# MihailMihov/simd-raytracer

Hardware: AMD Instinct MI355X
Metric: Mrays/s (intersect invocations per second), hw09/scene5 dragon 1920x1080 1spp (higher is better)
Workload: dtype f32; 1 GPU; BASELINE configs[1]: scenes/hw09/scene5.crtscene 1920x1080 1spp max_ray_depth=5 (primary + shadow + reflection rays), kd_tree_simd_accel semantics; rays_per_frame=2726485, primary_rays=2073600, parallelism=bucket-tiles x1

## Files before the change

### simd-raytracer_amd/csrc/accel.hpp

```cpp
#pragma once

#include <hip/hip_runtime.h>

#include <cstdlib>
#include <mutex>
#include <string>
#include <vector>

#include "abi_guard.hpp"
#include "kernels.hpp"
#include "stream.hpp"
#include "build.hpp"
#include "dev_mem.hpp"
#include "frame_plan.hpp"
#include "order_judge.hpp"
#include "update_plan.hpp"

struct rtk_knobs {
    uint32_t slice_min_tris = rtk::kSliceMinTrisDefault;
    bool shadow_exit = true;
    bool skip_unlit_shadow = true;
    bool bundle_cull = true;
    bool auto_trials = true;
    bool cost_feedback = true;
// ... 24 lines not shown
    int stream_batch = 0;
    int stream_mem_gb = 96;
    int stream_side_below = 2;
    bool first_frame_prior = true;
    bool fast_occluders = true;
    bool camera_keeps_order = false;
    size_t views_launch_units = 131072;
    bool traversal_fast = false;
    size_t adaptive_chunk_pixels = size_t(1) << 20;

    static rtk_knobs from_env() {
        rtk_knobs k;
        auto geti = [](const char *name, long &out) { const char *e = std::getenv(name); if (!e || !*e) return false; out = std::atol(e); return true; };
        long v;
        if (geti("RTK_SLICE_MIN_TRIS", v) && v > 0) k.slice_min_tris = uint32_t(v);
        if (geti("RTK_SHADOW_EARLY_EXIT", v)) k.shadow_exit = v != 0;
        if (geti("RTK_SKIP_UNLIT_SHADOW", v)) k.skip_unlit_shadow = v != 0;
        if (geti("RTK_BUNDLE_CULL", v)) k.bundle_cull = v != 0;
        if (geti("RTK_AUTO_TRIALS", v)) k.auto_trials = v != 0;
        if (geti("RTK_COST_FEEDBACK", v)) k.cost_feedback = v != 0;
        if (geti("RTK_COST_RESORT_EVERY", v) && v > 0) { k.resort_every = unsigned(v); k.resort_max = 0; }
        if (geti("RTK_COST_RESORT_MAX", v) && v >= 0 && v <= (1l << 30)) k.resort_max = unsigned(v);
        if (geti("RTK_COST_JUDGE", v)) k.judge = v != 0;
        if (geti("RTK_COST_JUDGE_FORCE", v) && v >= rtk::kJudgeByScore && v <= rtk::kJudgeAlwaysKeep) k.judge_force = int(v);
        if (geti("RTK_LIGHT_BELOW_CYCLES", v) && v >= 0) k.light_cycles = uint32_t(v);
        if (geti("RTK_ORDER_FLOOR_CYCLES", v) && v >= 0) k.order_floor_cycles = uint32_t(v);
        if (geti("RTK_REPACK", v)) k.repack = v != 0;
        if (geti("RTK_RASTER_TILES", v)) k.raster_tiles = v != 0;
        if (geti("RTK_REPACK_FULL_BOUNDS", v)) k.repack_full_bounds = v != 0;
        if (geti("RTK_REPACK_SKIP_BITS2", v) && v >= 0 && v <= 22) k.repack_skip_bits2 = int(v);
        if (geti("RTK_REPACK_DIRS3", v)) k.repack_dirs3 = v != 0;
        if (geti("RTK_REPACK_SKIP_BITS", v) && v >= 0 && v <= 14) k.repack_skip_bits = int(v);
        if (geti("RTK_STREAM_SCALAR_SURV", v)) k.stream_scalar_surv = v != 0;
        if (geti("RTK_BATCH_SCALAR_SURV", v)) k.batch_scalar_surv = v != 0;
        if (geti("RTK_REPACK_TRACE", v) && (v == RTK_TRACE_AUTO || v == RTK_TRACE_WAVE || v == RTK_TRACE_LANE)) k.repack_trace = int(v);
        if (geti("RTK_GROUP8_BELOW_BLOCKS", v) && v >= 0) k.group8_below = size_t(v);
        if (geti("RTK_STREAM_NODE_FACTOR", v) && v >= 1) k.stream_node_factor = int(v);
        if (geti("RTK_STREAM_DEEP_LEVEL", v)) k.stream_deep_level = int(v);
        if (geti("RTK_STREAM_DEEP_MODE", v)) k.stream_deep_mode = int(v);
        if (geti("RTK_AUTO_MIN_LANES", v) && v > 0 && v <= 64) k.auto_min_lanes = uint32_t(v);
        if (geti("RTK_STREAM_SORT_FROM", v)) k.stream_sort_from = int(v);
        if (geti("RTK_STREAM_DEBUG", v)) k.stream_debug = v != 0;
        if (geti("RTK_STREAM_SIDE", v)) k.stream_side = v != 0;
        if (geti("RTK_TRAVERSAL_FAST", v)) k.traversal_fast = v != 0;
        if (geti("RTK_FIRST_FRAME_PRIOR", v)) k.first_frame_prior = v != 0;
        if (geti("RTK_STREAM_SLICES", v) && (v == 0 || v == 1 || v == 2 || v == 4)) k.stream_slices = int(v);
        if (geti("RTK_STREAM_BATCH", v) && v >= 0 && v <= 4096) k.stream_batch = int(v);
// ... 330 lines not shown
```

### simd-raytracer_amd/csrc/api_frame.hip

```cpp
#include <cmath>
#include <cstdio>
#include <cstring>
#include <mutex>

#include "accel.hpp"
#include "stream_plan.hpp"

namespace rtk {

int frame_geom(const rtk_accel *a, const rtk_render_params *p, FrameGeom &g) {
    if (!a || !p) return fail(RTK_ERR_INVALID, "null accel or params");
    const int64_t w = p->width > 0 ? p->width : a->scene.width;
    const int64_t h = p->height > 0 ? p->height : a->scene.height;
    if (w <= 0 || h <= 0 || w > 65536 || h > 65536) return fail(RTK_ERR_INVALID, "image size must be in [1, 65536]");
    if (p->spp < 1) return fail(RTK_ERR_INVALID, "spp must be >= 1");
    if (p->max_ray_depth < 0 || p->max_ray_depth > kMaxRayDepth)
        return fail(RTK_ERR_INVALID, "max_ray_depth must be in [0, 16]");
    if (p->diffuse_rays < 0 || p->diffuse_rays > 32767) return fail(RTK_ERR_INVALID, "diffuse_rays must be in [0, 32767]");
    if (!valid_frame_mode(p->trace_mode)) return fail(RTK_ERR_INVALID, "unknown trace_mode");
    if (p->sample_begin < 0 || p->sample_count < 0 || p->sample_begin >= p->spp ||
        int64_t(p->sample_begin) + p->sample_count > p->spp)
        return fail(RTK_ERR_INVALID, "sample_begin / sample_count must select samples inside [0, spp)");
    if (p->sample_count == 0 && p->sample_begin != 0) return fail(RTK_ERR_INVALID, "sample_count == 0 means all samples: sample_begin must be 0");
    g.sample_begin = p->sample_begin;
// ... 257 lines not shown
    }
    RTK_TRY(join_lanes(a, lanes, s));
    S.ws = a->ws;
    RTK_HIP_AS(launch_stream_overflow_reset(S, s), "launch overflow reset");
    dev::RenderArgs F = A;
    F.only_if = a->ws.ctrl + dev::kCtrlOverflow;
    RTK_HIP_AS(launch_render(F, RTK_TRACE_GROUP4, p->collect_stats != 0, general, s), "launch fallback k_render");
    RTK_TRY(release_stream_ws(a, s));
    if (a->knobs.stream_debug) {
        uint32_t h[dev::kCtrlWords];
        (void)hipStreamSynchronize(s);
        (void)hipMemcpy(h, a->ws.ctrl, sizeof(h), hipMemcpyDeviceToHost);
        std::fprintf(stderr, "[rtk stream] node_cap %u hit_cap %u overflow %u; nodes per level:", a->ws.node_cap, a->ws.hit_cap, h[dev::kCtrlOverflow]);
        for (int l = 0; l <= p->max_ray_depth + 1; ++l) std::fprintf(stderr, " %u", l == 0 ? unsigned(n_root) : h[dev::kCtrlNodeCount + l]);
        std::fprintf(stderr, "; hits:");
        for (int l = 0; l <= p->max_ray_depth; ++l) std::fprintf(stderr, " %u", h[dev::kCtrlHitCount + l]);
        std::fprintf(stderr, "\n");
    }
    return RTK_OK;
}

int ensure_feedback_ws(rtk_accel *a, rtk_cost_feedback &fb, const FrameGeom &g, size_t units, hipStream_t s) {
    if (fb.judge.get() == nullptr) {
        RTK_MEM(fb.judge.reserve(kJudgeWords));
        RTK_HIP(hipMemsetAsync(fb.judge.get(), 0, kJudgeWords * sizeof(uint32_t), s));
    }
    if (fb.state.units >= units) return RTK_OK;
    const uint32_t bk = g.bucket;
    const uint64_t tx = (uint64_t(a->scene.width > 0 ? a->scene.width : 0) + bk - 1) / bk, ty = (uint64_t(a->scene.height > 0 ? a->scene.height : 0) + bk - 1) / bk;
    const size_t cap = fb.state.capacity(units, &fb == &a->fb, g.blocks_of(tx * ty));
    RTK_MEM(fb.cost.reserve(cap));
    RTK_MEM(fb.order.reserve(2 * (2 * cap + 4) + 8));
    RTK_MEM(fb.bins.reserve(cap));
    fb.state.units = cap;
    return RTK_OK;
}

struct ListSet { uint32_t *order, *hdr, *wg_list; };
ListSet list_set(rtk_cost_feedback &fb, int k, size_t units) {
    uint32_t *const order = fb.order.get() + size_t(k) * (2 * fb.state.units + 4);
    return {order, order + units, order + units + 4};
}

int read_back_count(rtk_cost_feedback &fb, const ListSet &L, hipStream_t s) {
    RTK_MEM(fb.nwgs_host.reserve(1));
    RTK_MEM(fb.nwgs_ev.ensure());
    RTK_HIP(hipMemcpyAsync(fb.nwgs_host.get(), L.hdr, sizeof(uint32_t), hipMemcpyDeviceToHost, s));
    RTK_HIP(hipEventRecord(fb.nwgs_ev.get(), s));
    return RTK_OK;
}

int launch_sort(rtk_accel *a, rtk_cost_feedback &fb, int k, int frame_mode, size_t units, hipStream_t s, int champion) {
    const ListSet L = list_set(fb, k, units);
    RTK_HIP_AS(launch_order_by_cost(fb.cost.get(), fb.bins.get(), L.order, L.wg_list, L.hdr, uint32_t(units),
                                    frame_mode == RTK_TRACE_GROUP4 ? a->knobs.light_cycles >> 4 : 0u, a->knobs.order_floor_cycles >> 4, 4u, s,
                                    a->knobs.judge ? fb.judge.get() : nullptr, champion),
               "launch k_order_by_cost");
    fb.sorts += 1;
    return read_back_count(fb, L, s);
}

int launch_judge(rtk_accel *a, rtk_cost_feedback &fb, int read_set, size_t units, hipStream_t s) {
    const ListSet R = list_set(fb, read_set, units), O = list_set(fb, read_set ^ 1, units);
    RTK_HIP_AS(launch_judge_order(fb.judge.get(), R.order, O.order, uint32_t(2 * units + 4), a->knobs.judge_force, s), "launch k_judge_order");
    fb.judges += 1;
    fb.state.rearm_count();
    return read_back_count(fb, R, s);
}

int order_launch(rtk_accel *a, rtk_cost_feedback &fb, const rtk_render_params *p, const FrameGeom &g, dev::RenderArgs &A, int frame_mode,
                 size_t units, hipStream_t s, OrderState::Step &step) {
    uint64_t sig[5];
    shape_sig(g, p->spp, p->max_ray_depth, p->diffuse_rays, sig);
    sig[3] = (uint64_t(uint32_t(g.bucket)) << 32) | (uint64_t(uint32_t(g.sample_end - g.sample_begin) & 0xFFFFu) << 16) | uint32_t(p->trace_mode);
    sig[4] = A.regions ? ((1ull << 63) | (uint64_t(A.n_regions) << 32) | uint64_t(A.n_units))
                       : (A.views ? uint64_t(A.n_views) : 0ull);
    RTK_TRY(ensure_feedback_ws(a, fb, g, units, s));
    step = fb.state.step(sig, frame_mode, p->collect_stats != 0, A.regions != nullptr,
                         {a->knobs.first_frame_prior, a->knobs.resort_every, a->knobs.resort_max});
    fb.list_units = units;
    const ListSet L = list_set(fb, step.read_set, units);
    if (step.prior)
        RTK_HIP_AS(launch_block_prior(A, fb.bins.get(), L.order, L.wg_list, L.hdr,
                                      reinterpret_cast<uint32_t *>(A.counters + kPriorScratchWord), 4u, s), "launch k_block_prior");
    if (step.sort_front) RTK_TRY(launch_sort(a, fb, step.read_set, frame_mode, units, s, kChampionNone));
    if (step.use_order) { A.order_in = L.order; A.order_hdr = L.hdr; A.wg_list = L.wg_list; }
    if (&fb == &a->fb) a->cnt.after_order(step);
    A.cost_out = fb.cost.get();
    return RTK_OK;
}

int render_megakernel(rtk_accel *a, rtk_cost_feedback &fb, const rtk_render_params *p, const FrameGeom &g, dev::RenderArgs &A, bool general,
                      hipStream_t s) {
    const size_t units = A.regions ? size_t(A.n_units) : (A.views ? g.blocks() * A.n_views : g.blocks());
    A.n_units = uint32_t(units);
    const int frame_mode = OrderState::frame_mode(p->trace_mode, units, a->knobs.group8_below);
    OrderState::Step step = {};
    if (a->knobs.cost_feedback && units > 0 && units <= 0x7FFFFFFFull) {
        const int rc = order_launch(a, fb, p, g, A, frame_mode, units, s, step);
        if (rc != RTK_OK) { fb.forget(); return rc; }
    }
    unsigned n_wgs = 0;
    if (A.wg_list != nullptr) {
        bool ready = false;
        if (fb.state.awaits_count() && !(ready = hipEventQuery(fb.nwgs_ev.get()) == hipSuccess)) (void)hipGetLastError();
        n_wgs = fb.state.workgroups(ready, fb.nwgs_host.get());
    }
    int rc = RTK_OK;
    const bool judged = step.judge && a->knobs.judge && units <= 0x7FFFFFF0ull / 2;
    if (a->knobs.judge && (judged || step.sort_behind)) {
        n_wgs = 0;
        const hipError_t es = launch_stamp(fb.judge.get(), s);
        if (es != hipSuccess) rc = hip_fail(es, "launch k_stamp");
    }
    const hipError_t e = rc == RTK_OK ? launch_render(A, frame_mode, p->collect_stats != 0, general, s, n_wgs) : hipSuccess;
    if (e != hipSuccess) rc = hip_fail(e, "launch k_render");
    if (rc == RTK_OK && judged) rc = launch_judge(a, fb, step.read_set, units, s);
    if (rc == RTK_OK && step.sort_behind)
        rc = launch_sort(a, fb, step.write_set, frame_mode, units, s, judged ? kChampionLeave : kChampionScore);
    if (rc != RTK_OK) fb.forget();
    return rc;
}

}

dev::RenderArgs frame_args(const rtk_accel *a, const rtk_render_params *p, const FrameGeom &g, const rtk_view &cam, float *d_out) {
    dev::RenderArgs A = scene_args(a, p->collect_stats);
    camera_args(cam, p, g, A);
    A.max_depth = p->max_ray_depth; A.diffuse_rays = p->diffuse_rays;
    A.gi_div_f = static_cast<float>(p->diffuse_rays + 1);
    A.sample_begin = g.sample_begin; A.sample_end = g.sample_end;
    A.shadow_bias = p->shadow_bias; A.reflection_bias = p->reflection_bias; A.refraction_bias = p->refraction_bias;
    A.bucket = g.bucket; A.tiles_x = g.tiles_x; A.tiles_y = g.tiles_y; A.n_buckets = g.n_buckets;
    A.blocks_per_bucket_side = g.blocks_side; A.buckets_per_rank = g.buckets_per_rank;
    A.rank = g.rank; A.world = g.world; A.compact = g.world > 1 ? 1 : 0; A.skew_q = g.skew_q;
    A.out = d_out; A.counters = counters_now(a);
    return A;
}

namespace {

int render_frame_body(rtk_accel *a, const rtk_render_params *p, const FrameGeom &g, const rtk_view &cam, float *d_out, hipStream_t s, bool steady) {
// ... 588 lines not shown
```

### simd-raytracer_amd/csrc/frame_plan.hpp

```cpp
#pragma once

#include <cstddef>
#include <cstdint>
#include <cstring>

#include "../../include/rtk.h"

namespace rtk {

struct FrameGeom {
    uint32_t width, height, bucket, tiles_x, tiles_y, n_buckets, blocks_side, buckets_per_rank;
    uint32_t skew_q;
    int rank, world;
    int sample_begin, sample_end;
    uint64_t blocks_of(uint64_t buckets) const { return buckets * blocks_side * blocks_side; }
    size_t blocks() const { return size_t(blocks_of(buckets_per_rank)); }
};

inline void shape_sig(const FrameGeom &g, int spp, int max_ray_depth, int diffuse_rays, uint64_t out[3]) {
    out[0] = (uint64_t(uint32_t(g.width)) << 32) | uint32_t(g.height);
    out[1] = (uint64_t(uint32_t(g.rank)) << 32) | uint32_t(g.world);
    out[2] = (uint64_t(uint32_t(spp)) << 32) | (uint64_t(uint32_t(max_ray_depth)) << 16) | uint32_t(diffuse_rays);
}

// ... 3 lines not shown
    uint64_t sig[3] = {0, 0, 0};
    int state = 0;

    static bool applies(int trace_mode, bool forks, bool stats) { return trace_mode == RTK_TRACE_AUTO && forks && !stats; }
    bool same(const uint64_t s[3]) const { return std::memcmp(s, sig, sizeof(sig)) == 0; }
    bool waiting(const uint64_t s[3]) const { return state == 3 && same(s); }
    void verdict(float t_stream, float t_mega) { state = t_mega < t_stream ? 5 : 4; }
    void abandon() { state = 0; }
    Step next(const uint64_t s[3], bool trials_on) {
        if (!same(s)) { std::memcpy(sig, s, sizeof(sig)); state = 0; }
        if (!trials_on) return {true, kNoRecord};
        switch (state) {
            case 0: state = 1; return {true, kPipelinePair};
            case 1: state = 2; return {false, kNoRecord};
            case 2: state = 3; return {false, kMegakernelPair};
            case 5: return {false, kNoRecord};
            default: return {true, kNoRecord};
        }
    }
};

struct OrderState {
    struct Knobs { bool first_frame_prior; unsigned resort_every; unsigned resort_max = 0; };
    struct Step { bool prior, resort, use_order, sort_front, sort_behind; int read_set, write_set; bool judge = false; };
    size_t units = 0;
    uint64_t sig[5] = {0, 0, 0, 0, 0};
    bool valid = false;
    bool order_valid = false;
    unsigned age = 0;
    bool nwgs_pending = false, nwgs_known = false;
    int set = 0;
    bool presorted = false;
    unsigned sorts = 0;

    void forget() { valid = false; order_valid = false; age = 0; nwgs_pending = false; nwgs_known = false; set = 0; presorted = false; sorts = 0; }

    void restart_schedule(unsigned resort_every) {
        sorts = 0;
        if (!presorted && resort_every > 0 && age >= resort_every) age = resort_every - 1;
    }

    unsigned interval(const Knobs &k) const {
        uint64_t iv = k.resort_every;
        for (unsigned i = 3; i <= sorts && iv < k.resort_max; ++i) iv *= 2;
        return (k.resort_max > k.resort_every && iv > k.resort_max) ? k.resort_max : unsigned(iv);
    }

    static int frame_mode(int trace_mode, size_t n_units, size_t group8_below) {
        if (trace_mode == RTK_TRACE_TWOPASS) return RTK_TRACE_GROUP4;
        return trace_mode != RTK_TRACE_AUTO ? trace_mode : (n_units < group8_below ? RTK_TRACE_GROUP8 : RTK_TRACE_GROUP4);
    }

    size_t capacity(size_t n_units, bool is_frame_table, uint64_t native) {
        if (units >= n_units) return units;
        size_t cap = n_units;
        if (is_frame_table && units == 0 && native > cap && native <= (1ull << 24)) cap = size_t(native);
        units = 0; valid = false; order_valid = false;
        return cap;
    }

    Step step(const uint64_t s[5], int mode, bool stats, bool regions, const Knobs &k) {
        const bool same_shape = valid && std::memcmp(s, sig, sizeof(sig)) == 0;
        if (!same_shape) { order_valid = false; set = 0; presorted = false; sorts = 0; }
        Step r = {!same_shape && k.first_frame_prior && mode == RTK_TRACE_GROUP4 && !stats && !regions, false, false, false, false, 0, 0, false};
        if (same_shape) {
            r.resort = !order_valid || age >= interval(k);
            if (r.resort) {
                r.sort_front = !presorted;
                r.judge = presorted;
                if (presorted) set ^= 1;
                presorted = false;
                order_valid = true; age = 0; nwgs_known = false; nwgs_pending = true;
                sorts += 1;
            }
            age += 1;
            r.sort_behind = age >= interval(k);
            presorted = r.sort_behind;
        }
        r.use_order = r.prior || same_shape;
        r.read_set = set; r.write_set = set ^ 1;
        std::memcpy(sig, s, sizeof(sig));
        valid = true;
        return r;
    }

    void rearm_count() { if (order_valid) { nwgs_pending = true; nwgs_known = false; } }

    bool awaits_count() const { return order_valid && nwgs_pending; }
    unsigned workgroups(bool ready, const uint32_t *host_word) {
        if (!order_valid) return 0;
        if (nwgs_pending && ready) { nwgs_pending = false; nwgs_known = true; }
        return nwgs_known && !nwgs_pending ? *host_word : 0;
    }
};

struct CounterState {
    struct Step { int current; bool fill, carry; };
    int current = 0;
    bool other_zero = false;
    const void *stream = nullptr;
// ... 40 lines not shown
```

### simd-raytracer_amd/csrc/kernels.hip

```cpp
#include <hip/hip_runtime.h>

#include "kernels.hpp"
#include "order_judge.hpp"
#include "trace.hip.hpp"
#include "shade.hip.hpp"

namespace rtk {
namespace dev {

template <int MODE, bool STATS, bool LDS_NODES>
__global__ __launch_bounds__(256) void k_intersect(IntersectArgs A) {
    extern __shared__ __attribute__((aligned(16))) unsigned char smem[];
    DevNode *lds_nodes = reinterpret_cast<DevNode *>(smem);
    if (LDS_NODES) stage_nodes(A.tree.nodes, A.tree.n_nodes, lds_nodes);

    const size_t slot = (size_t)blockIdx.x * blockDim.x + threadIdx.x;
    const bool active = slot < A.n;
    size_t i = (active && A.perm != nullptr) ? (size_t)A.perm[slot] : slot;
    uint32_t raster_w = A.raster_w;
    if (A.verdict != nullptr) {
        if (A.verdict[16] != 0u) return;
        raster_w = A.verdict[15];
        if (raster_w < 64u || (raster_w & 7u) != 0u || (size_t)raster_w * 16u > A.n) raster_w = 0u;
    }
// ... 866 lines not shown
    const unsigned long long a = acc[i], c = cur[i];
    acc[i] = longest ? (a < c ? c : a) : a + c;
}
}

hipError_t launch_counters_fold(const unsigned long long *cur, unsigned long long *acc, hipStream_t s) {
    hipLaunchKernelGGL(dev::k_counters_fold, dim3(1), dim3(256), 0, s, cur, acc);
    return hipGetLastError();
}

namespace dev {
__device__ __forceinline__ uint32_t cost_bin(uint32_t c) {
    c |= 1u;
    const uint32_t e = 31u - (uint32_t)__clz((int)c);
    const uint32_t m = e >= 3u ? (c >> (e - 3u)) & 7u : (c << (3u - e)) & 7u;
    return e * 8u + m;
}
__global__ __launch_bounds__(1024) void k_order_by_cost(const uint32_t *cost, uint8_t *bins, uint32_t *order, uint32_t *wg_list,
                                                        uint32_t *hdr, uint32_t n, uint32_t light_below, uint32_t floor_below,
                                                        uint32_t pack, uint32_t *judge, int champion) {
    if (judge != nullptr && threadIdx.x == 0u) {
        const unsigned long long now = __builtin_amdgcn_s_memrealtime();
        const unsigned long long t0 = *reinterpret_cast<const unsigned long long *>(judge + kJudgeStampLo);
        if (champion != kChampionLeave) judge[kJudgeChampion] = champion == kChampionScore ? judge_score(t0, now) : 0u;
    }
    __shared__ uint32_t hist[256];
    __shared__ uint32_t start[256];
    __shared__ uint32_t wg_hist[2][256], wg_base[2][256];
    __shared__ uint32_t n_single_sh;
    const uint32_t light_bin = light_below > 0u ? cost_bin(light_below) : 0u;
    const uint32_t floor_raw = floor_below > 0u ? cost_bin(floor_below) : 0u;
    const uint32_t floor_bin = floor_raw < light_bin ? floor_raw : light_bin;
    constexpr uint32_t kBatch = 8;
    for (uint32_t i = threadIdx.x; i < 256u; i += blockDim.x) { hist[i] = 0u; wg_hist[0][i] = 0u; wg_hist[1][i] = 0u; }
    __syncthreads();
    for (uint32_t base = 0; base < n; base += blockDim.x * kBatch) {
        uint32_t c[kBatch];
#pragma unroll
        for (uint32_t k = 0; k < kBatch; ++k) {
            const uint32_t i = base + k * blockDim.x + threadIdx.x;
            c[k] = i < n ? cost[i] : 0u;
        }
#pragma unroll
        for (uint32_t k = 0; k < kBatch; ++k) {
            const uint32_t i = base + k * blockDim.x + threadIdx.x;
            uint32_t b = i < n ? cost_bin(c[k]) : 0u;
            if (b < floor_bin) b = 0u;
// ... 66 lines not shown
    __syncthreads();
    for (uint32_t w = threadIdx.x; w < n_wgs; w += blockDim.x) {
        const bool packed = w >= n_single;
        const uint32_t at = packed ? n_single + (w - n_single) * pack : w;
        const uint32_t blk = order[at];
        uint32_t key = (uint32_t)bins[blk];
        if (packed && key != 0u) key = key + 8u < 255u ? key + 8u : 255u;
        const uint32_t pos = atomicAdd(&wg_base[packed ? 1 : 0][key], 1u);
        wg_list[pos] = packed ? (0x80000000u | at) : blk;
    }
}
}

hipError_t launch_order_by_cost(const uint32_t *cost, uint8_t *bins, uint32_t *order, uint32_t *wg_list, uint32_t *hdr, uint32_t n,
                                uint32_t light_below, uint32_t floor_below, uint32_t pack, hipStream_t s, uint32_t *judge, int champion) {
    if (n == 0u) return hipSuccess;
    if (pack == 0u) return hipErrorInvalidValue;
    hipLaunchKernelGGL(dev::k_order_by_cost, dim3(1), dim3(1024), 0, s, cost, bins, order, wg_list, hdr, n, light_below, floor_below, pack,
                       judge, champion);
    return hipGetLastError();
}

namespace dev {
__global__ __launch_bounds__(64) void k_stamp(unsigned long long *stamp) {
    if (threadIdx.x == 0u) *stamp = __builtin_amdgcn_s_memrealtime();
}
}

hipError_t launch_stamp(uint32_t *judge, hipStream_t s) {
    if (judge == nullptr) return hipErrorInvalidValue;
    hipLaunchKernelGGL(dev::k_stamp, dim3(1), dim3(64), 0, s, reinterpret_cast<unsigned long long *>(judge + kJudgeStampLo));
    return hipGetLastError();
}

namespace dev {
__global__ __launch_bounds__(1024) void k_judge_order(uint32_t *judge, uint32_t *read_set, const uint32_t *other_set, uint32_t words, int force) {
    __shared__ uint32_t take_sh;
    if (threadIdx.x == 0u) {
        const unsigned long long now = __builtin_amdgcn_s_memrealtime();
        const unsigned long long t0 = *reinterpret_cast<const unsigned long long *>(judge + kJudgeStampLo);
        const Verdict v = judge_order({judge[kJudgeChampion], judge_score(t0, now)}, force);
        judge[kJudgeChampion] = v.after.champion;
        judge[kJudgeChallenger] = v.after.challenger;
        judge[v.take ? kJudgeTaken : kJudgeRejected] += 1u;
        take_sh = v.take ? 1u : 0u;
    }
    __syncthreads();
    if (take_sh != 0u) return;
    uint32_t done = 0u;
    if (((reinterpret_cast<uintptr_t>(read_set) | reinterpret_cast<uintptr_t>(other_set)) & 15u) == 0u) {
        const uint32_t quads = words >> 2;
        const uint4 *src = reinterpret_cast<const uint4 *>(other_set);
        uint4 *dst = reinterpret_cast<uint4 *>(read_set);
        constexpr uint32_t kBatch = 4;
        for (uint32_t base = 0; base < quads; base += blockDim.x * kBatch) {
            uint4 v[kBatch];
#pragma unroll
            for (uint32_t k = 0; k < kBatch; ++k) {
                const uint32_t i = base + k * blockDim.x + threadIdx.x;
                if (i < quads) v[k] = src[i];
            }
#pragma unroll
            for (uint32_t k = 0; k < kBatch; ++k) {
                const uint32_t i = base + k * blockDim.x + threadIdx.x;
                if (i < quads) dst[i] = v[k];
            }
        }
        done = quads << 2;
    }
    for (uint32_t i = done + threadIdx.x; i < words; i += blockDim.x) read_set[i] = other_set[i];
}
}

hipError_t launch_judge_order(uint32_t *judge, uint32_t *read_set, const uint32_t *other_set, uint32_t words, int force, hipStream_t s) {
    if (judge == nullptr || read_set == nullptr || other_set == nullptr || read_set == other_set) return hipErrorInvalidValue;
    if (words == 0u) return hipSuccess;
    hipLaunchKernelGGL(dev::k_judge_order, dim3(1), dim3(1024), 0, s, judge, read_set, other_set, words, force);
    return hipGetLastError();
}

hipError_t launch_camera_rays(const dev::RenderArgs &A, int sample, rtk_ray *d_rays, hipStream_t s) {
    const size_t n = (size_t)A.width * A.height;
    if (n == 0) return hipSuccess;
    hipLaunchKernelGGL(dev::k_camera_rays, dim3((unsigned)((n + 255) / 256)), dim3(256), 0, s, A, sample, d_rays);
    return hipGetLastError();
}

hipError_t launch_region_rays(const dev::RenderArgs &A, int sample, uint64_t first, uint32_t n, rtk_ray *d_rays, uint32_t *d_ids, hipStream_t s) {
    if (n == 0u) return hipSuccess;
    if (A.regions == nullptr || A.n_regions == 0u) return hipErrorInvalidValue;
    hipLaunchKernelGGL(dev::k_region_rays, dim3((n + 255u) / 256u), dim3(256), 0, s, A, sample, first, n, d_rays, d_ids);
    return hipGetLastError();
}

hipError_t launch_region_accumulate(const dev::RenderArgs &A, uint64_t first, uint32_t n, const float *d_rgb, bool start, bool divide, hipStream_t s) {
    if (n == 0u) return hipSuccess;
    if (A.regions == nullptr || A.n_regions == 0u) return hipErrorInvalidValue;
    hipLaunchKernelGGL(dev::k_region_accumulate, dim3((n + 255u) / 256u), dim3(256), 0, s, A, first, n, d_rgb, start ? 1 : 0, divide ? 1 : 0);
    return hipGetLastError();
}
// ... 29 lines not shown
```

### simd-raytracer_amd/csrc/kernels.hpp

```cpp
#pragma once

#include <hip/hip_runtime.h>

#include "rtk_internal.hpp"
#include "counters.hpp"

namespace rtk {

constexpr int kMaxRayDepth = 16;
constexpr unsigned long long kCriticalMinTicks = 1000;
constexpr uint32_t kSliceMinTrisDefault = 33;
constexpr size_t kMaxNodeLdsBytes = 48 * 1024;

}

#include "trace.hip.hpp"
#include "regions_plan.hpp"

namespace rtk {
namespace dev {

__host__ __device__ inline uint32_t rank_bucket(uint32_t rank, uint32_t local, uint32_t world, uint32_t skew_q) {
    if (skew_q == 0u) return rank + local * world;
    const uint32_t by = local / skew_q, m = local % skew_q;
// ... 64 lines not shown
    const RegionEntry *regions;
    uint32_t n_regions;

    __device__ __forceinline__ size_t out_index(uint32_t local_bucket, uint32_t lx, uint32_t ly, uint32_t px,
                                                uint32_t py) const {
        return compact ? (((size_t)local_bucket * bucket + ly) * bucket + lx) : ((size_t)py * width + px);
    }
};

struct AssembleArgs {
    const float *gathered;
    float *rgb;
    uint32_t width, height, bucket, tiles_x, world, buckets_per_rank, skew_q;
};

}

hipError_t launch_intersect(const dev::IntersectArgs &A, int mode, bool stats, hipStream_t s);
hipError_t launch_render(const dev::RenderArgs &A, int mode, bool stats, bool forks, hipStream_t s, unsigned n_workgroups = 0);
enum : int { kChampionNone = 0, kChampionScore = 1, kChampionLeave = 2 };
hipError_t launch_order_by_cost(const uint32_t *cost, uint8_t *bins , uint32_t *order, uint32_t *wg_list ,
                                uint32_t *hdr , uint32_t n, uint32_t light_below, uint32_t floor_below, uint32_t pack,
                                hipStream_t s, uint32_t *judge = nullptr, int champion = kChampionNone);
hipError_t launch_stamp(uint32_t *judge, hipStream_t s);
hipError_t launch_judge_order(uint32_t *judge, uint32_t *read_set, const uint32_t *other_set, uint32_t words, int force, hipStream_t s);
hipError_t launch_block_prior(const dev::RenderArgs &A, uint8_t *cls, uint32_t *order, uint32_t *wg_list, uint32_t *hdr,
                              uint32_t *scratch, uint32_t pack, hipStream_t s);
hipError_t launch_counters_fold(const unsigned long long *cur, unsigned long long *acc, hipStream_t s);
hipError_t launch_assemble(const dev::AssembleArgs &A, hipStream_t s);
hipError_t launch_camera_rays(const dev::RenderArgs &A, int sample, rtk_ray *d_rays, hipStream_t s);
hipError_t launch_to_rgb8(const float *d_rgb, size_t n, uint8_t *d_out, hipStream_t s);
hipError_t launch_frame_to_texels(const float *d_rgb, size_t n, uint8_t *d_out, hipStream_t s);
hipError_t launch_region_rays(const dev::RenderArgs &A, int sample, uint64_t first, uint32_t n, rtk_ray *d_rays, uint32_t *d_ids, hipStream_t s);
hipError_t launch_region_accumulate(const dev::RenderArgs &A, uint64_t first, uint32_t n, const float *d_rgb, bool start, bool divide, hipStream_t s);
hipError_t launch_add_word(unsigned long long *dst, const unsigned long long *src, hipStream_t s);

}
```

### simd-raytracer_amd/csrc/order_judge.hpp

```cpp
#pragma once

#include <cstdint>

#if defined(__HIPCC__) || defined(__CUDACC__)
#define RTK_JUDGE_FN __host__ __device__ inline
#else
#define RTK_JUDGE_FN inline
#endif

namespace rtk {

enum : int { kJudgeByScore = 0, kJudgeAlwaysTake = 1, kJudgeAlwaysKeep = 2 };

enum : uint32_t {
    kJudgeStampLo = 0, kJudgeStampHi = 1,
    kJudgeChampion = 2,
    kJudgeChallenger = 3,
    kJudgeTaken = 4, kJudgeRejected = 5,
    kJudgeWords = 6
};

RTK_JUDGE_FN uint32_t judge_score(uint64_t frame_start, uint64_t behind_start) {
    if (frame_start == 0 || behind_start <= frame_start) return 0u;
    const uint64_t d = behind_start - frame_start;
    return d > 0xFFFFFFFFull ? 0xFFFFFFFFu : uint32_t(d);
}

struct JudgeScores { uint32_t champion, challenger; };
struct Verdict {
    bool take;
    JudgeScores after;
};

RTK_JUDGE_FN Verdict judge_order(JudgeScores s, int force) {
    bool take = s.champion == 0u || s.challenger == 0u || s.challenger <= s.champion;
    if (force == kJudgeAlwaysTake) take = true;
    if (force == kJudgeAlwaysKeep) take = false;
    return {take, {take ? s.challenger : s.champion, s.challenger}};
}

}
```

### simd-raytracer_amd/csrc/phases.hip.hpp

```cpp
#pragma once

#include <hip/hip_runtime.h>

#include <cstdint>

namespace rtk {
namespace dev {

enum PhaseSlot : int {
    PH_TOTAL = 0,
    PH_TRACE, PH_N_TRACE,
    PH_STEPS,
    PH_N_SMALL, PH_T_SMALL, PH_C_SMALL,
    PH_N_BIG, PH_T_BIG, PH_C_BIG,
    PH_PROLOGUE, PH_TO_FIRST_TRACE, PH_FIRST_TRACE, PH_AFTER_FIRST_TRACE,
    PH_CHUNKS, PH_SURV, PH_CTRIS,
    PH_RT0, PH_RT1,
    PH_WG,
    PH_WAIT,
    PH_TR0, PH_TR1, PH_TR2, PH_TR3, PH_TR4, PH_TR5,
    PH_KIND0, PH_KIND1, PH_KIND2, PH_KIND3, PH_KIND4, PH_KIND5,
    PH_C_BUND, PH_C_LIST,
    PH_OWN,
    PH_STG_N,
    PH_STG_W1, PH_STG_L1, PH_STG_W2, PH_STG_L2, PH_STG_W3, PH_STG_L3,
    PH_STG_L4,
    PH_SLOTS
};

#ifdef RTK_DEBUG_PHASES
constexpr bool kPhases = true;
#define RTK_PHASES_ONLY(...) __VA_ARGS__
#else
constexpr bool kPhases = false;
#define RTK_PHASES_ONLY(...)
#endif

struct PhaseTallies { uint32_t v[PH_SLOTS] = {}; };
struct Stamp {
    RTK_PHASES_ONLY(unsigned long long t0;)
    static __device__ __forceinline__ Stamp now() { return Stamp{RTK_PHASES_ONLY(__builtin_readcyclecounter())}; }
};

struct Probe {
    RTK_PHASES_ONLY(PhaseTallies *t = nullptr;)
    __device__ __forceinline__ void add(const int slot, const uint32_t n) const { RTK_PHASES_ONLY(if (t) t->v[slot] += n;) }
    __device__ __forceinline__ void since(const Stamp s, const int slot) const { RTK_PHASES_ONLY(add(slot, (uint32_t)(__builtin_readcyclecounter() - s.t0));) }
    __device__ __forceinline__ void tri() const { add(PH_STG_N, 1u); }
    __device__ __forceinline__ void alive(const int w, const unsigned long long m) const { add(w, 1u); add(w + 1, (uint32_t)__popcll(m)); }
    __device__ __forceinline__ void accepted(const unsigned long long m) const { add(PH_STG_L4, (uint32_t)__popcll(m)); }
    __device__ __forceinline__ void cull_pass(const unsigned long long surv, const uint32_t tris) const { add(PH_CHUNKS, 1u); add(PH_SURV, (uint32_t)__popcll(surv)); add(PH_CTRIS, tris); }
    __device__ __forceinline__ void node_step() const { add(PH_STEPS, 1u); }
    __device__ __forceinline__ void list_pass(const unsigned long long cand, const Stamp s) const { add(PH_STEPS, (uint32_t)__popcll(cand)); since(s, PH_C_LIST); }
    __device__ __forceinline__ void leaf(const bool sliced, const uint32_t tris, const Stamp s) const {
        since(s, sliced ? PH_C_BIG : PH_C_SMALL); add(sliced ? PH_N_BIG : PH_N_SMALL, 1u); add(sliced ? PH_T_BIG : PH_T_SMALL, tris);
    }
};
#define RTK_PHASE_TALLIES_OF_SLICECTX                   \
    RTK_PHASES_ONLY(PhaseTallies phase_tallies = {};)   \
    __device__ __forceinline__ Probe probe() { return Probe{RTK_PHASES_ONLY(&phase_tallies)}; }

struct FrameProbe {
    RTK_PHASES_ONLY(unsigned long long entry, rt0, begin = 0, first_trace = 0, after_first = 0, tr0 = 0, w0 = 0;)
    static __device__ __forceinline__ FrameProbe enter() { return FrameProbe{RTK_PHASES_ONLY(__builtin_readcyclecounter(), __builtin_amdgcn_s_memrealtime())}; }
    __device__ __forceinline__ void prologue_done() { RTK_PHASES_ONLY(begin = __builtin_readcyclecounter();) }
    __device__ __forceinline__ void trace_begins() { RTK_PHASES_ONLY(tr0 = __builtin_readcyclecounter(); if (first_trace == 0) first_trace = tr0;) }
    __device__ __forceinline__ void trace_returned() { RTK_PHASES_ONLY(w0 = __builtin_readcyclecounter();) }
    __device__ __forceinline__ void trace_done(const Probe p, const bool burst, const bool sliced, const uint32_t burst_plog, const bool in_root) {
        RTK_PHASES_ONLY(
        p.since(Stamp{w0}, PH_WAIT);
        if (burst && sliced) p.t->v[PH_OWN] = (uint32_t)(w0 - tr0);
        for (int i = 0; i < 6; ++i) if (p.t->v[PH_N_TRACE] == (uint32_t)i) {
            p.t->v[PH_TR0 + i] = (uint32_t)(__builtin_readcyclecounter() - tr0);
            p.t->v[PH_KIND0 + i] = burst ? 100u + burst_plog : (uint32_t)__popcll(__builtin_amdgcn_ballot_w64(in_root));
        }
        p.since(Stamp{tr0}, PH_TRACE); p.add(PH_N_TRACE, 1u);
        if (after_first == 0) after_first = __builtin_readcyclecounter();)
    }
    __device__ __forceinline__ void write(const Probe p, const uint32_t lane, float *o) const {
        RTK_PHASES_ONLY(
        const unsigned long long now = __builtin_readcyclecounter(), rt1 = __builtin_amdgcn_s_memrealtime();
        float vals[PH_SLOTS];
        for (int i = 0; i < PH_SLOTS; ++i) vals[i] = (float)p.t->v[i];
        vals[PH_TOTAL] = (float)(now - begin);
        vals[PH_PROLOGUE] = (float)(begin - entry);
        vals[PH_TO_FIRST_TRACE] = (float)(first_trace - begin);
        vals[PH_FIRST_TRACE] = (float)(after_first - first_trace);
        vals[PH_AFTER_FIRST_TRACE] = (float)(now - after_first);
        vals[PH_RT0] = (float)(rt0 & 0xFFFFFFull);
        vals[PH_RT1] = (float)(rt1 & 0xFFFFFFull);
        vals[PH_WG] = (float)blockIdx.x;
        float v = 0.f;
        for (int i = 0; i < PH_SLOTS; ++i) v = (lane == (uint32_t)i) ? vals[i] : v;
        o[0] = v; o[1] = 0.f; o[2] = 0.f;)
    }
};

}
}
```

Measured before the change: 16060 Mrays/s.

## Judge cost-ordered tile lists on a three-frame median with trial confirmation

Replaces the single-frame champion/challenger timing judgement for cost-sorted tile orders with a three-frame score ring and median. A newly adopted order is put on trial and is dropped back to the previous list if its median frame time is worse. A first-frame tolerance of about 1/16 is added when a confirmation will follow. This is meant to stop noisy single-frame timings from locking in a worse work order, at the cost of extra tiny stamp/score/confirm kernel launches per frame and possible list copy-backs. A debug-only hardware-id probe lane is also added.

Measured after the change: 15460 Mrays/s. -3.7%, worse.

```diff
diff --git a/simd-raytracer_amd/csrc/accel.hpp b/simd-raytracer_amd/csrc/accel.hpp
--- a/simd-raytracer_amd/csrc/accel.hpp
+++ b/simd-raytracer_amd/csrc/accel.hpp
@@ -70,7 +70,7 @@
         if (geti("RTK_COST_RESORT_EVERY", v) && v > 0) { k.resort_every = unsigned(v); k.resort_max = 0; }
         if (geti("RTK_COST_RESORT_MAX", v) && v >= 0 && v <= (1l << 30)) k.resort_max = unsigned(v);
         if (geti("RTK_COST_JUDGE", v)) k.judge = v != 0;
-        if (geti("RTK_COST_JUDGE_FORCE", v) && v >= rtk::kJudgeByScore && v <= rtk::kJudgeAlwaysKeep) k.judge_force = int(v);
+        if (geti("RTK_COST_JUDGE_FORCE", v) && v >= rtk::kJudgeByScore && v <= rtk::kJudgeTakeThenDrop) k.judge_force = int(v);
         if (geti("RTK_LIGHT_BELOW_CYCLES", v) && v >= 0) k.light_cycles = uint32_t(v);
         if (geti("RTK_ORDER_FLOOR_CYCLES", v) && v >= 0) k.order_floor_cycles = uint32_t(v);
         if (geti("RTK_REPACK", v)) k.repack = v != 0;
diff --git a/simd-raytracer_amd/csrc/api_frame.hip b/simd-raytracer_amd/csrc/api_frame.hip
--- a/simd-raytracer_amd/csrc/api_frame.hip
+++ b/simd-raytracer_amd/csrc/api_frame.hip
@@ -303,8 +303,8 @@
 
 int ensure_feedback_ws(rtk_accel *a, rtk_cost_feedback &fb, const FrameGeom &g, size_t units, hipStream_t s) {
     if (fb.judge.get() == nullptr) {
-        RTK_MEM(fb.judge.reserve(kJudgeWords));
-        RTK_HIP(hipMemsetAsync(fb.judge.get(), 0, kJudgeWords * sizeof(uint32_t), s));
+        RTK_MEM(fb.judge.reserve(kJudgeBlockWords));
+        RTK_HIP(hipMemsetAsync(fb.judge.get(), 0, kJudgeBlockWords * sizeof(uint32_t), s));
     }
     if (fb.state.units >= units) return RTK_OK;
     const uint32_t bk = g.bucket;
@@ -341,10 +341,17 @@
     return read_back_count(fb, L, s);
 }
 
-int launch_judge(rtk_accel *a, rtk_cost_feedback &fb, int read_set, size_t units, hipStream_t s) {
+int launch_judge(rtk_accel *a, rtk_cost_feedback &fb, int read_set, size_t units, hipStream_t s, bool confirmable) {
     const ListSet R = list_set(fb, read_set, units), O = list_set(fb, read_set ^ 1, units);
-    RTK_HIP_AS(launch_judge_order(fb.judge.get(), R.order, O.order, uint32_t(2 * units + 4), a->knobs.judge_force, s), "launch k_judge_order");
+    RTK_HIP_AS(launch_judge_order(fb.judge.get(), R.order, O.order, uint32_t(2 * units + 4), a->knobs.judge_force, s, confirmable), "launch k_judge_order");
     fb.judges += 1;
+    fb.state.rearm_count();
+    return read_back_count(fb, R, s);
+}
+
+int launch_confirm(rtk_accel *a, rtk_cost_feedback &fb, int read_set, size_t units, hipStream_t s) {
+    const ListSet R = list_set(fb, read_set, units), O = list_set(fb, read_set ^ 1, units);
+    RTK_HIP_AS(launch_confirm_order(fb.judge.get(), R.order, O.order, uint32_t(2 * units + 4), a->knobs.judge_force, s), "launch k_confirm_order");
     fb.state.rearm_count();
     return read_back_count(fb, R, s);
 }
@@ -388,17 +395,25 @@
         n_wgs = fb.state.workgroups(ready, fb.nwgs_host.get());
     }
     int rc = RTK_OK;
-    const bool judged = step.judge && a->knobs.judge && units <= 0x7FFFFFF0ull / 2;
-    if (a->knobs.judge && (judged || step.sort_behind)) {
+    const bool fits = units <= 0x7FFFFFF0ull / 2;
+    const bool judged = step.judge && a->knobs.judge && fits;
+    const bool confirmed = step.confirm && a->knobs.judge && fits && !judged;
+    const bool scored = a->knobs.judge && (judged || confirmed || step.sort_behind || step.scored);
+    if (scored) {
         n_wgs = 0;
-        const hipError_t es = launch_stamp(fb.judge.get(), s);
+        const hipError_t es = launch_stamp(fb.judge.get(), s, step.ring_clear);
         if (es != hipSuccess) rc = hip_fail(es, "launch k_stamp");
     }
     const hipError_t e = rc == RTK_OK ? launch_render(A, frame_mode, p->collect_stats != 0, general, s, n_wgs) : hipSuccess;
     if (e != hipSuccess) rc = hip_fail(e, "launch k_render");
-    if (rc == RTK_OK && judged) rc = launch_judge(a, fb, step.read_set, units, s);
+    if (rc == RTK_OK && judged) rc = launch_judge(a, fb, step.read_set, units, s, step.judge_on_trial);
+    if (rc == RTK_OK && confirmed) rc = launch_confirm(a, fb, step.read_set, units, s);
+    if (rc == RTK_OK && scored && !judged && !confirmed && !step.sort_behind) {
+        const hipError_t ek = launch_score(fb.judge.get(), s);
+        if (ek != hipSuccess) rc = hip_fail(ek, "launch k_score");
+    }
     if (rc == RTK_OK && step.sort_behind)
-        rc = launch_sort(a, fb, step.write_set, frame_mode, units, s, judged ? kChampionLeave : kChampionScore);
+        rc = launch_sort(a, fb, step.write_set, frame_mode, units, s, (judged || confirmed) ? kChampionLeave : kChampionScore);
     if (rc != RTK_OK) fb.forget();
     return rc;
 }
diff --git a/simd-raytracer_amd/csrc/frame_plan.hpp b/simd-raytracer_amd/csrc/frame_plan.hpp
--- a/simd-raytracer_amd/csrc/frame_plan.hpp
+++ b/simd-raytracer_amd/csrc/frame_plan.hpp
@@ -49,7 +49,11 @@
 
 struct OrderState {
     struct Knobs { bool first_frame_prior; unsigned resort_every; unsigned resort_max = 0; };
-    struct Step { bool prior, resort, use_order, sort_front, sort_behind; int read_set, write_set; bool judge = false; };
+    struct Step {
+        bool prior, resort, use_order, sort_front, sort_behind; int read_set, write_set; bool judge = false;
+        bool scored = false, ring_clear = false, confirm = false;
+        bool judge_on_trial = false;
+    };
     size_t units = 0;
     uint64_t sig[5] = {0, 0, 0, 0, 0};
     bool valid = false;
@@ -59,8 +63,14 @@
     int set = 0;
     bool presorted = false;
     unsigned sorts = 0;
+    bool judged_list = false;
+    bool scored_before = false;
+    static constexpr unsigned kScoreFrames = 3;
 
-    void forget() { valid = false; order_valid = false; age = 0; nwgs_pending = false; nwgs_known = false; set = 0; presorted = false; sorts = 0; }
+    void forget() {
+        valid = false; order_valid = false; age = 0; nwgs_pending = false; nwgs_known = false; set = 0; presorted = false; sorts = 0;
+        judged_list = false; scored_before = false;
+    }
 
     void restart_schedule(unsigned resort_every) {
         sorts = 0;
@@ -88,7 +98,7 @@
 
     Step step(const uint64_t s[5], int mode, bool stats, bool regions, const Knobs &k) {
         const bool same_shape = valid && std::memcmp(s, sig, sizeof(sig)) == 0;
-        if (!same_shape) { order_valid = false; set = 0; presorted = false; sorts = 0; }
+        if (!same_shape) { order_valid = false; set = 0; presorted = false; sorts = 0; judged_list = false; scored_before = false; }
         Step r = {!same_shape && k.first_frame_prior && mode == RTK_TRACE_GROUP4 && !stats && !regions, false, false, false, false, 0, 0, false};
         if (same_shape) {
             r.resort = !order_valid || age >= interval(k);
@@ -99,10 +109,18 @@
                 presorted = false;
                 order_valid = true; age = 0; nwgs_known = false; nwgs_pending = true;
                 sorts += 1;
+                judged_list = r.judge;
             }
             age += 1;
-            r.sort_behind = age >= interval(k);
+            const unsigned iv = interval(k);
+            r.sort_behind = age >= iv;
             presorted = r.sort_behind;
+            const bool on_trial = judged_list && iv >= kScoreFrames && age <= kScoreFrames;
+            r.confirm = on_trial && age == kScoreFrames;
+            r.judge_on_trial = r.judge && on_trial;
+            r.scored = on_trial || age + kScoreFrames > iv;
+            r.ring_clear = r.scored && !scored_before;
+            scored_before = r.scored;
         }
         r.use_order = r.prior || same_shape;
         r.read_set = set; r.write_set = set ^ 1;
diff --git a/simd-raytracer_amd/csrc/kernels.hip b/simd-raytracer_amd/csrc/kernels.hip
--- a/simd-raytracer_amd/csrc/kernels.hip
+++ b/simd-raytracer_amd/csrc/kernels.hip
@@ -912,7 +912,8 @@
     if (judge != nullptr && threadIdx.x == 0u) {
         const unsigned long long now = __builtin_amdgcn_s_memrealtime();
         const unsigned long long t0 = *reinterpret_cast<const unsigned long long *>(judge + kJudgeStampLo);
-        if (champion != kChampionLeave) judge[kJudgeChampion] = champion == kChampionScore ? judge_score(t0, now) : 0u;
+        if (champion == kChampionScore) judge[kJudgeChampion] = champion_score(judge + kJudgeRing, judge_score(t0, now));
+        if (champion == kChampionNone) { judge[kJudgeChampion] = 0u; ring_clear(judge + kJudgeRing); }
     }
     __shared__ uint32_t hist[256];
     __shared__ uint32_t start[256];
@@ -1025,31 +1026,34 @@
 }
 
 namespace dev {
-__global__ __launch_bounds__(64) void k_stamp(unsigned long long *stamp) {
-    if (threadIdx.x == 0u) *stamp = __builtin_amdgcn_s_memrealtime();
-}
-}
-
-hipError_t launch_stamp(uint32_t *judge, hipStream_t s) {
-    if (judge == nullptr) return hipErrorInvalidValue;
-    hipLaunchKernelGGL(dev::k_stamp, dim3(1), dim3(64), 0, s, reinterpret_cast<unsigned long long *>(judge + kJudgeStampLo));
-    return hipGetLastError();
-}
-
-namespace dev {
-__global__ __launch_bounds__(1024) void k_judge_order(uint32_t *judge, uint32_t *read_set, const uint32_t *other_set, uint32_t words, int force) {
-    __shared__ uint32_t take_sh;
+__global__ __launch_bounds__(64) void k_stamp(uint32_t *judge, int clear) {
+    if (threadIdx.x == 0u) {
+        if (clear != 0) ring_clear(judge + kJudgeRing);
+        *reinterpret_cast<unsigned long long *>(judge + kJudgeStampLo) = __builtin_amdgcn_s_memrealtime();
+    }
+}
+__global__ __launch_bounds__(64) void k_score(uint32_t *judge) {
     if (threadIdx.x == 0u) {
         const unsigned long long now = __builtin_amdgcn_s_memrealtime();
-        const unsigned long long t0 = *reinterpret_cast<const unsigned long long *>(judge + kJudgeStampLo);
-        const Verdict v = judge_order({judge[kJudgeChampion], judge_score(t0, now)}, force);
-        judge[kJudgeChampion] = v.after.champion;
-        judge[kJudgeChallenger] = v.after.challenger;
-        judge[v.take ? kJudgeTaken : kJudgeRejected] += 1u;
-        take_sh = v.take ? 1u : 0u;
-    }
-    __syncthreads();
-    if (take_sh != 0u) return;
+        ring_push(judge + kJudgeRing, judge_score(*reinterpret_cast<const unsigned long long *>(judge + kJudgeStampLo), now));
+    }
+}
+}
+
+hipError_t launch_stamp(uint32_t *judge, hipStream_t s, bool ring_clear) {
+    if (judge == nullptr) return hipErrorInvalidValue;
+    hipLaunchKernelGGL(dev::k_stamp, dim3(1), dim3(64), 0, s, judge, ring_clear ? 1 : 0);
+    return hipGetLastError();
+}
+
+hipError_t launch_score(uint32_t *judge, hipStream_t s) {
+    if (judge == nullptr) return hipErrorInvalidValue;
+    hipLaunchKernelGGL(dev::k_score, dim3(1), dim3(64), 0, s, judge);
+    return hipGetLastError();
+}
+
+namespace dev {
+__device__ __forceinline__ void lists_back(uint32_t *read_set, const uint32_t *other_set, const uint32_t words) {
     uint32_t done = 0u;
     if (((reinterpret_cast<uintptr_t>(read_set) | reinterpret_cast<uintptr_t>(other_set)) & 15u) == 0u) {
         const uint32_t quads = words >> 2;
@@ -1073,12 +1077,57 @@
     }
     for (uint32_t i = done + threadIdx.x; i < words; i += blockDim.x) read_set[i] = other_set[i];
 }
-}
-
-hipError_t launch_judge_order(uint32_t *judge, uint32_t *read_set, const uint32_t *other_set, uint32_t words, int force, hipStream_t s) {
+__global__ __launch_bounds__(1024) void k_judge_order(uint32_t *judge, uint32_t *read_set, const uint32_t *other_set, uint32_t words, int force,
+                                                      int confirmable) {
+    __shared__ uint32_t take_sh;
+    if (threadIdx.x == 0u) {
+        const unsigned long long now = __builtin_amdgcn_s_memrealtime();
+        const unsigned long long t0 = *reinterpret_cast<const unsigned long long *>(judge + kJudgeStampLo);
+        const JudgeScores before = {judge[kJudgeChampion], judge_score(t0, now)};
+        const Verdict v = first_frame_order(before, force, confirmable != 0);
+        judge[kJudgeChampion] = v.after.champion;
+        judge[kJudgeChallenger] = v.after.challenger;
+        judge[v.take ? kJudgeTaken : kJudgeRejected] += 1u;
+        const Trial t = begin_trial(judge + kJudgeRing, before, v, force);
+        judge[kJudgeChampionBefore] = t.champion_before;
+        judge[kJudgeOnTrial] = t.on_trial;
+        take_sh = v.take ? 1u : 0u;
+    }
+    __syncthreads();
+    if (take_sh != 0u) return;
+    lists_back(read_set, other_set, words);
+}
+__global__ __launch_bounds__(1024) void k_confirm_order(uint32_t *judge, uint32_t *read_set, const uint32_t *other_set, uint32_t words, int force) {
+    __shared__ uint32_t drop_sh;
+    if (threadIdx.x == 0u) {
+        const unsigned long long now = __builtin_amdgcn_s_memrealtime();
+        const unsigned long long t0 = *reinterpret_cast<const unsigned long long *>(judge + kJudgeStampLo);
+        const Confirmed c = confirm_order(judge + kJudgeRing, {judge[kJudgeChampion], judge[kJudgeChallenger]},
+                                          {judge[kJudgeChampionBefore], judge[kJudgeOnTrial]}, judge_score(t0, now), force);
+        judge[kJudgeChampion] = c.after.champion;
+        judge[kJudgeChallenger] = c.after.challenger;
+        if (c.drop) { judge[kJudgeTaken] -= 1u; judge[kJudgeRejected] += 1u; }
+        judge[kJudgeOnTrial] = 0u;
+        drop_sh = c.drop ? 1u : 0u;
+    }
+    __syncthreads();
+    if (drop_sh == 0u) return;
+    lists_back(read_set, other_set, words);
+}
+}
+
+hipError_t launch_confirm_order(uint32_t *judge, uint32_t *read_set, const uint32_t *other_set, uint32_t words, int force, hipStream_t s) {
     if (judge == nullptr || read_set == nullptr || other_set == nullptr || read_set == other_set) return hipErrorInvalidValue;
     if (words == 0u) return hipSuccess;
-    hipLaunchKernelGGL(dev::k_judge_order, dim3(1), dim3(1024), 0, s, judge, read_set, other_set, words, force);
+    hipLaunchKernelGGL(dev::k_confirm_order, dim3(1), dim3(1024), 0, s, judge, read_set, other_set, words, force);
+    return hipGetLastError();
+}
+
+hipError_t launch_judge_order(uint32_t *judge, uint32_t *read_set, const uint32_t *other_set, uint32_t words, int force, hipStream_t s,
+                              bool confirmable) {
+    if (judge == nullptr || read_set == nullptr || other_set == nullptr || read_set == other_set) return hipErrorInvalidValue;
+    if (words == 0u) return hipSuccess;
+    hipLaunchKernelGGL(dev::k_judge_order, dim3(1), dim3(1024), 0, s, judge, read_set, other_set, words, force, confirmable ? 1 : 0);
     return hipGetLastError();
 }
 
diff --git a/simd-raytracer_amd/csrc/kernels.hpp b/simd-raytracer_amd/csrc/kernels.hpp
--- a/simd-raytracer_amd/csrc/kernels.hpp
+++ b/simd-raytracer_amd/csrc/kernels.hpp
@@ -110,8 +110,11 @@
 hipError_t launch_order_by_cost(const uint32_t *cost, uint8_t *bins , uint32_t *order, uint32_t *wg_list ,
                                 uint32_t *hdr , uint32_t n, uint32_t light_below, uint32_t floor_below, uint32_t pack,
                                 hipStream_t s, uint32_t *judge = nullptr, int champion = kChampionNone);
-hipError_t launch_stamp(uint32_t *judge, hipStream_t s);
-hipError_t launch_judge_order(uint32_t *judge, uint32_t *read_set, const uint32_t *other_set, uint32_t words, int force, hipStream_t s);
+hipError_t launch_stamp(uint32_t *judge, hipStream_t s, bool ring_clear = false);
+hipError_t launch_score(uint32_t *judge, hipStream_t s);
+hipError_t launch_confirm_order(uint32_t *judge, uint32_t *read_set, const uint32_t *other_set, uint32_t words, int force, hipStream_t s);
+hipError_t launch_judge_order(uint32_t *judge, uint32_t *read_set, const uint32_t *other_set, uint32_t words, int force, hipStream_t s,
+                              bool confirmable = false);
 hipError_t launch_block_prior(const dev::RenderArgs &A, uint8_t *cls, uint32_t *order, uint32_t *wg_list, uint32_t *hdr,
                               uint32_t *scratch, uint32_t pack, hipStream_t s);
 hipError_t launch_counters_fold(const unsigned long long *cur, unsigned long long *acc, hipStream_t s);
diff --git a/simd-raytracer_amd/csrc/order_judge.hpp b/simd-raytracer_amd/csrc/order_judge.hpp
--- a/simd-raytracer_amd/csrc/order_judge.hpp
+++ b/simd-raytracer_amd/csrc/order_judge.hpp
@@ -10,7 +10,7 @@
 
 namespace rtk {
 
-enum : int { kJudgeByScore = 0, kJudgeAlwaysTake = 1, kJudgeAlwaysKeep = 2 };
+enum : int { kJudgeByScore = 0, kJudgeAlwaysTake = 1, kJudgeAlwaysKeep = 2, kJudgeTakeThenDrop = 3 };
 
 enum : uint32_t {
     kJudgeStampLo = 0, kJudgeStampHi = 1,
@@ -19,6 +19,11 @@
     kJudgeTaken = 4, kJudgeRejected = 5,
     kJudgeWords = 6
 };
+enum : uint32_t {
+    kJudgeRing = kJudgeWords, kJudgeRingCount = kJudgeRing + 3, kJudgeChampionBefore, kJudgeOnTrial,
+    kJudgeBlockWords
+};
+constexpr uint32_t kJudgeFrames = 3;
 
 RTK_JUDGE_FN uint32_t judge_score(uint64_t frame_start, uint64_t behind_start) {
     if (frame_start == 0 || behind_start <= frame_start) return 0u;
@@ -34,9 +39,58 @@
 
 RTK_JUDGE_FN Verdict judge_order(JudgeScores s, int force) {
     bool take = s.champion == 0u || s.challenger == 0u || s.challenger <= s.champion;
-    if (force == kJudgeAlwaysTake) take = true;
+    if (force == kJudgeAlwaysTake || force == kJudgeTakeThenDrop) take = true;
     if (force == kJudgeAlwaysKeep) take = false;
     return {take, {take ? s.challenger : s.champion, s.challenger}};
 }
 
+RTK_JUDGE_FN Verdict first_frame_order(JudgeScores s, int force, bool confirmable) {
+    if (confirmable && force == kJudgeByScore && s.champion != 0u && s.challenger != 0u) {
+        const bool take = uint64_t(s.challenger) <= uint64_t(s.champion) + (s.champion >> 4);
+        return {take, {take ? s.challenger : s.champion, s.challenger}};
+    }
+    return judge_order(s, force);
 }
+
+RTK_JUDGE_FN void ring_clear(uint32_t *ring) { ring[kJudgeFrames] = 0u; }
+RTK_JUDGE_FN void ring_push(uint32_t *ring, uint32_t score) {
+    if (score == 0u) return;
+    const uint32_t n = ring[kJudgeFrames];
+    ring[n % kJudgeFrames] = score;
+    ring[kJudgeFrames] = n == 0xFFFFFFFFu ? n - (kJudgeFrames - 1u) : n + 1u;
+}
+RTK_JUDGE_FN uint32_t ring_median(const uint32_t *ring) {
+    const uint32_t n = ring[kJudgeFrames], a = ring[0], b = ring[1], c = ring[2];
+    if (n == 0u) return 0u;
+    if (n == 1u) return a;
+    if (n == 2u) return a < b ? a : b;
+    const uint32_t lo = a < b ? a : b, hi = a < b ? b : a;
+    return c < lo ? lo : (c > hi ? hi : c);
+}
+
+RTK_JUDGE_FN uint32_t champion_score(uint32_t *ring, uint32_t frame) {
+    ring_push(ring, frame);
+    return frame == 0u ? 0u : ring_median(ring);
+}
+
+struct Trial { uint32_t champion_before, on_trial; };
+RTK_JUDGE_FN Trial begin_trial(uint32_t *ring, JudgeScores before, Verdict v, int force) {
+    ring_clear(ring);
+    if (v.take) ring_push(ring, before.challenger);
+    const bool by_score = force == kJudgeByScore && before.champion != 0u && before.challenger != 0u;
+    return {before.champion, (v.take && (by_score || force == kJudgeTakeThenDrop)) ? 1u : 0u};
+}
+
+struct Confirmed { bool drop; JudgeScores after; };
+RTK_JUDGE_FN Confirmed confirm_order(uint32_t *ring, JudgeScores now, Trial t, uint32_t frame, int force) {
+    ring_push(ring, frame);
+    if (t.on_trial == 0u) return {false, now};
+    const uint32_t median = ring_median(ring);
+    bool drop = ring[kJudgeFrames] >= kJudgeFrames && t.champion_before != 0u && median > t.champion_before;
+    if (force == kJudgeTakeThenDrop) drop = true;
+    if (force == kJudgeAlwaysTake) drop = false;
+    if (drop) { ring_clear(ring); return {true, {t.champion_before, median != 0u ? median : now.challenger}}; }
+    return {false, {median != 0u ? median : now.champion, median != 0u ? median : now.challenger}};
+}
+
+}
diff --git a/simd-raytracer_amd/csrc/phases.hip.hpp b/simd-raytracer_amd/csrc/phases.hip.hpp
--- a/simd-raytracer_amd/csrc/phases.hip.hpp
+++ b/simd-raytracer_amd/csrc/phases.hip.hpp
@@ -27,6 +27,9 @@
     PH_STG_L4,
     PH_SLOTS
 };
+constexpr int PH_HW_ID = PH_SLOTS;
+constexpr int PH_LANES = PH_SLOTS + 1;
+static_assert(PH_LANES <= 64, "one value per lane of the owner wave");
 
 #ifdef RTK_DEBUG_PHASES
 constexpr bool kPhases = true;
@@ -61,8 +64,12 @@
     __device__ __forceinline__ Probe probe() { return Probe{RTK_PHASES_ONLY(&phase_tallies)}; }
 
 struct FrameProbe {
-    RTK_PHASES_ONLY(unsigned long long entry, rt0, begin = 0, first_trace = 0, after_first = 0, tr0 = 0, w0 = 0;)
-    static __device__ __forceinline__ FrameProbe enter() { return FrameProbe{RTK_PHASES_ONLY(__builtin_readcyclecounter(), __builtin_amdgcn_s_memrealtime())}; }
+    RTK_PHASES_ONLY(unsigned long long entry, rt0; uint32_t hw; unsigned long long begin = 0, first_trace = 0, after_first = 0, tr0 = 0, w0 = 0;)
+    static __device__ __forceinline__ FrameProbe enter() { return FrameProbe{RTK_PHASES_ONLY(__builtin_readcyclecounter(), __builtin_amdgcn_s_memrealtime(), hw_id())}; }
+    static __device__ __forceinline__ uint32_t hw_id() {
+        RTK_PHASES_ONLY(return ((uint32_t)__builtin_amdgcn_s_getreg(4 | (31 << 11)) & 0xFFFFu) | ((uint32_t)__builtin_amdgcn_s_getreg(20 | (3 << 11)) << 16);)
+        return 0u;
+    }
     __device__ __forceinline__ void prologue_done() { RTK_PHASES_ONLY(begin = __builtin_readcyclecounter();) }
     __device__ __forceinline__ void trace_begins() { RTK_PHASES_ONLY(tr0 = __builtin_readcyclecounter(); if (first_trace == 0) first_trace = tr0;) }
     __device__ __forceinline__ void trace_returned() { RTK_PHASES_ONLY(w0 = __builtin_readcyclecounter();) }
@@ -80,7 +87,7 @@
     __device__ __forceinline__ void write(const Probe p, const uint32_t lane, float *o) const {
         RTK_PHASES_ONLY(
         const unsigned long long now = __builtin_readcyclecounter(), rt1 = __builtin_amdgcn_s_memrealtime();
-        float vals[PH_SLOTS];
+        float vals[PH_LANES];
         for (int i = 0; i < PH_SLOTS; ++i) vals[i] = (float)p.t->v[i];
         vals[PH_TOTAL] = (float)(now - begin);
         vals[PH_PROLOGUE] = (float)(begin - entry);
@@ -90,8 +97,9 @@
         vals[PH_RT0] = (float)(rt0 & 0xFFFFFFull);
         vals[PH_RT1] = (float)(rt1 & 0xFFFFFFull);
         vals[PH_WG] = (float)blockIdx.x;
+        vals[PH_HW_ID] = (float)hw;
         float v = 0.f;
-        for (int i = 0; i < PH_SLOTS; ++i) v = (lane == (uint32_t)i) ? vals[i] : v;
+        for (int i = 0; i < PH_LANES; ++i) v = (lane == (uint32_t)i) ? vals[i] : v;
         o[0] = v; o[1] = 0.f; o[2] = 0.f;)
     }
 };
```
